# lichunshang/vision-enhanced-lidar-odometry

Hardware: AMD Instinct MI355X
Metric: scan-pairs/sec + achieved HBM GB/s, 120k-pt HDL-64E frame-to-frame ICP (higher is better)
Workload: dtype f32 association / f64 residuals+solve

## Files before the change

### vision-enhanced-lidar-odometry_amd/csrc/velo_kernels.h

```cpp
#pragma once
#include <hip/hip_runtime.h>
#include <stdint.h>

#include "velo_device_math.h"

#ifndef VELO_DEF_LOAD
#define VELO_DEF_LOAD 0
#endif
#ifndef VELO_DEF_ASSOC
#define VELO_DEF_ASSOC 0
#endif
#ifndef VELO_DEF_LMA
#define VELO_DEF_LMA 0
#endif
#ifndef VELO_DEF_LMB
#define VELO_DEF_LMB 0
#endif

namespace velo {

constexpr int kWave = 64;
constexpr int kNumAcc = 28;
constexpr int kEvalThreads = 256;
constexpr int kMaxEvalBlocks = 512;
// ... 2565 lines not shown
__device__ __forceinline__ int visual_block_eval3(const PoseEval& P, const VisualMatch& m, int slot, double& r0, double& r1, double& r2, double J[18]) {
    r0 = 0.0; r1 = 0.0; r2 = 0.0;
    int d;
    if (slot == 0) {
        if (!WITH_2D2D || (m.d1 && m.d2)) {
            const double a[3] = {m.p3_1[0], m.p3_1[1], m.p3_1[2]}, s[3] = {m.p3_2[0], m.p3_2[1], m.p3_2[2]};
            double rl[3];
            res_3d3d(P.fwd, P.t, a, s, rl, J);
            r0 = rl[0]; r1 = rl[1]; r2 = rl[2]; d = 3;
        } else {
            const double a[2] = {m.p2_1[0], m.p2_1[1]}, s[2] = {m.p2_2[0], m.p2_2[1]}, tc[3] = {m.t_cam[0], m.t_cam[1], m.t_cam[2]};
            double rl[1];
            res_2d2d(P.fwd, P.t, a, s, tc, rl, J);
            r0 = rl[0]; d = 1;
        }
    } else {
        const double tc[3] = {m.t_cam[0], m.t_cam[1], m.t_cam[2]};
        double rl[2];
        if (slot == 1) {
            const double a[3] = {m.p3_1[0], m.p3_1[1], m.p3_1[2]}, s[2] = {m.p2_2[0], m.p2_2[1]};
            res_3d2d(P.fwd, P.t, a, s, tc, rl, J);
        } else {
            const double a[3] = {m.p3_2[0], m.p3_2[1], m.p3_2[2]}, s[2] = {m.p2_1[0], m.p2_1[1]};
            res_2d3d(P.inv, P.t, a, s, tc, rl, J);
        }
        r0 = rl[0]; r1 = rl[1]; d = 2;
    }
    return d;
}
__device__ __forceinline__ int visual_block_eval(const PoseEval& P, const VisualMatch& m, int slot, double r[3], double J[18]) {
    double r0, r1, r2;
    const int d = visual_block_eval3(P, m, slot, r0, r1, r2, J);
    r[0] = r0; r[1] = r1; r[2] = r2;
    return d;
}

__device__ __forceinline__ void visual_gate_body(const double* __restrict__ xdev, const VisualParams& V, const VisualMatch* __restrict__ matches, int n, int iter,
                                                 unsigned char* __restrict__ flags, int* __restrict__ counts, const int i) {
    if (i >= n) return;
    double x[6];
#pragma unroll
    for (int k = 0; k < 6; k++) x[k] = xdev[k];
    PoseEval P;
    pose_eval_init(x, &P, true);
    const VisualMatch m = matches[i];
    unsigned char f0 = 0, f1 = 0, f2 = 0;
    bool stop = false;
    double r[3], J[18];
    const double it = (double)iter;
    if (m.d1 && m.d2) {
        visual_block_eval(P, m, 0, r, J);
        const double th2 = V.th_3d3d * V.outlier_reject / it * V.th_3d3d * V.outlier_reject / it;
        if (iter > 1 && r[0] * r[0] + r[1] * r[1] + r[2] * r[2] > th2) stop = true; else f0 = 1 + 0;
    }
    if (!stop && !m.d1 && !m.d2 && V.enable_2d2d) {
        visual_block_eval(P, m, 0, r, J);
        if (iter > 1 && fabs(r[0]) > V.th_2d2d * V.outlier_reject / it) stop = true; else f0 = 1 + 3;
    }
    if (V.enable_3d2d) {
        const double th2 = V.th_3d2d * V.outlier_reject / it * V.th_3d2d * V.outlier_reject / it;
        if (!stop && m.d1) {
            visual_block_eval(P, m, 1, r, J);
            if (iter > 1 && r[0] * r[0] + r[1] * r[1] > th2) stop = true; else f1 = 1 + 1;
        }
        if (!stop && m.d2) {
            visual_block_eval(P, m, 2, r, J);
            if (iter > 1 && r[0] * r[0] + r[1] * r[1] > th2) stop = true; else f2 = 1 + 2;
        }
    }
    flags[3 * i + 0] = f0; flags[3 * i + 1] = f1; flags[3 * i + 2] = f2;
    if (counts) {
        const int nb = (f0 ? 1 : 0) + (f1 ? 1 : 0) + (f2 ? 1 : 0);
        const int nr = (f0 ? (f0 - 1 == VELO_RESIDUAL_3D3D ? 3 : 1) : 0) + (f1 ? 2 : 0) + (f2 ? 2 : 0);
        if (nb) { atomicAdd(&counts[0], nb); atomicAdd(&counts[1], nr); }
    }
}
__global__ void visual_gate_kernel(const double* __restrict__ xdev, VisualParams V, const VisualMatch* __restrict__ matches, int n, int iter,
                                   unsigned char* __restrict__ flags, int* __restrict__ counts)
#if VELO_DEF_LMA
{
    visual_gate_body(xdev, V, matches, n, iter, flags, counts, (int)(blockIdx.x * blockDim.x + threadIdx.x));
}
#else
;
#endif
constexpr int kGateJobs = 8;
struct GateBatch {
    const double* x[kGateJobs]; const VisualMatch* m[kGateJobs]; unsigned char* flags[kGateJobs]; int* counts[kGateJobs]; int n[kGateJobs];
    VisualParams V; int iter;
};
__global__ void __launch_bounds__(128) visual_gate_batch_kernel(GateBatch G)
#if VELO_DEF_LMA
{
    const int j = blockIdx.y;
    visual_gate_body(G.x[j], G.V, G.m[j], G.n[j], G.iter, G.flags[j], G.counts[j], (int)(blockIdx.x * 128 + threadIdx.x));
}
#else
;
#endif

enum { PHASE_INIT = 0, PHASE_CAND = 1 };
struct LMParams {
    int max_num_iterations, max_invalid;
    double function_tolerance, gradient_tolerance, parameter_tolerance;
    double initial_radius, max_radius, min_radius, min_relative_decrease, min_diag, max_diag;
};
struct LMState {
    double x[6];
    double xc[6];
    double H[21];
    double g[6];
    double cost;
    double scale[6];
    double diag[6];
    double radius, decrease, x_norm, model_change, step_norm;
    double initial_cost;
    int reuse_diag, invalid, iter, evals, done, termination, phase, n_valid;
};
static_assert(sizeof(LMState) % 8 == 0 && sizeof(LMState) / 8 <= 64, "the state is copied by one wave, one 8-byte word per lane");

__device__ __forceinline__ int tri(int i, int j) { return i * 6 - (i * (i - 1)) / 2 + (j - i); }

struct LMEvalPoint {
    double M[4][9];
    double t[3];
    double x[6];
    int done;
    int pad;
};
static_assert(sizeof(LMEvalPoint) % 8 == 0 && sizeof(LMEvalPoint) / 8 <= 64, "the eval point is copied by one wave, one 8-byte word per lane");

__device__ __forceinline__ void eval_point_column(const double x[6], int done, int col, LMEvalPoint* P) {
    if (col < 3) {
        PoseRot R;
        pose_rot_init(x, &R);
        const double e[3] = {col == 0 ? 1.0 : 0.0, col == 1 ? 1.0 : 0.0, col == 2 ? 1.0 : 0.0};
        D3 m[3];
        rotate_point(R, e, m);
#pragma unroll
        for (int k = 0; k < 3; k++) {
            P->M[0][3 * k + col] = m[k].a;
#pragma unroll
            for (int j = 0; j < 3; j++) P->M[1 + j][3 * k + col] = m[k].v[j];
        }
    } else if (col == 3) {
#pragma unroll
        for (int k = 0; k < 3; k++) P->t[k] = x[3 + k];
#pragma unroll
        for (int k = 0; k < 6; k++) P->x[k] = x[k];
        P->done = done; P->pad = 0;
    }
}

__device__ __forceinline__ void res_3dpd_mat(const double (*M)[9], const double t[3], const double p[3], const double n[3], const double v0[3],
                                             double* r, double J[6]) {
    double m[3];
#pragma unroll
    for (int k = 0; k < 3; k++) m[k] = (M[0][3 * k] * p[0] + M[0][3 * k + 1] * p[1] + M[0][3 * k + 2] * p[2]) + (t[k] - v0[k]);
    *r = m[0] * n[0] + m[1] * n[1] + m[2] * n[2];
#pragma unroll
    for (int j = 0; j < 3; j++) {
        double d[3];
#pragma unroll
        for (int k = 0; k < 3; k++) d[k] = M[1 + j][3 * k] * p[0] + M[1 + j][3 * k + 1] * p[1] + M[1 + j][3 * k + 2] * p[2];
        J[j] = d[0] * n[0] + d[1] * n[1] + d[2] * n[2];
    }
    J[3] = n[0]; J[4] = n[1]; J[5] = n[2];
}

struct EvalArgs {
    const LMState* __restrict__ state;
    const LMEvalPoint* __restrict__ pt;
    const double* __restrict__ x_override;
    const float4* __restrict__ cp;
    const float4* __restrict__ cn;
    const float4* __restrict__ cv0;
    int q_begin, q_end;
    const VisualMatch* __restrict__ vm;
    const unsigned char* __restrict__ vflags;
    int n_matches;
    double loss_a_3dpd, w_3dpd;
    VisualParams V;
    double* __restrict__ partials;
    int vis_row0;
    double* __restrict__ rows_r;
    double* __restrict__ rows_J;
    const int* __restrict__ row_offset_vis;
    const int* __restrict__ row_offset_icp;
    unsigned long long* __restrict__ trace;
    int trace_eval;
};

constexpr int kStatTypes = 5;
constexpr int kStatBins = 65536;
struct StatWork {
    unsigned long long prefix[kStatTypes];
    long long k[kStatTypes];
    long long count[kStatTypes];
    double sum[kStatTypes];
    double cost;
};
__global__ void __launch_bounds__(256)
residual_norms_kernel(const double* __restrict__ xdev, EvalArgs A, double* __restrict__ vals, signed char* __restrict__ types,
                      double* __restrict__ part )
#if VELO_DEF_LMA
{
    __shared__ PoseEval s_P;
    __shared__ double s_red[256];
    if (threadIdx.x == 0) {
        double x[6];
        for (int k = 0; k < 6; k++) x[k] = xdev[k];
        pose_eval_init(x, &s_P, true);
    }
    __syncthreads();
    const int n_vis = 3 * A.n_matches, nq = A.q_end - A.q_begin;
    const int i = blockIdx.x * blockDim.x + threadIdx.x;
    double v = 0.0, sq = 0.0;
    int type = -1;
    if (i < n_vis) {
        const unsigned char f = A.vflags[i];
        if (f) {
            const VisualMatch m = A.vm[i / 3];
            double r0, r1, r2, J[18];
            const int d = visual_block_eval3(s_P, m, i % 3, r0, r1, r2, J);
            type = f - 1;
            if (d == 3) { sq = r0 * r0 + r1 * r1 + r2 * r2; v = sqrt(sq); }
            else if (d == 2) { sq = r0 * r0 + r1 * r1; v = sqrt(sq); }
            else { sq = r0 * r0; v = fabs(r0); }
        }
    } else if (i < n_vis + nq) {
        const int qi = A.q_begin + (i - n_vis);
        const float4 cp = A.cp[qi];
        if (__float_as_int(cp.w)) {
            const float4 cn = A.cn[qi], c0 = A.cv0[qi];
            const double p[3] = {cp.x, cp.y, cp.z}, n[3] = {cn.x, cn.y, cn.z}, v0[3] = {c0.x, c0.y, c0.z};
            double r, J[6];
            res_3dpd(s_P.fwd, s_P.t, p, n, v0, &r, J);
            type = VELO_FUNCTOR_3DPD; sq = r * r; v = fabs(r);
        }
    }
    if (i < n_vis + nq) { vals[i] = v; types[i] = (signed char)type; }
    for (int t = 0; t <= kStatTypes; t++) {
        s_red[threadIdx.x] = (t < kStatTypes) ? (type == t ? v : 0.0) : sq;
        __syncthreads();
        for (int off = 128; off > 0; off >>= 1) { if ((int)threadIdx.x < off) s_red[threadIdx.x] += s_red[threadIdx.x + off]; __syncthreads(); }
        if (threadIdx.x == 0) part[(size_t)blockIdx.x * (kStatTypes + 1) + t] = s_red[0];
        __syncthreads();
    }
}
#else
;
#endif
__global__ void __launch_bounds__(256)
stats_hist_kernel(const double* __restrict__ vals, const signed char* __restrict__ types, int n, int pass, const StatWork* __restrict__ W, int* __restrict__ hist)
#if VELO_DEF_LMA
{
    const int i = blockIdx.x * blockDim.x + threadIdx.x;
    if (i >= n) return;
    const int t = types[i];
    if (t < 0) return;
    const unsigned long long b = (unsigned long long)__double_as_longlong(vals[i]);
    if (pass > 0 && (b >> (64 - 16 * pass)) != W->prefix[t]) return;
    atomicAdd(&hist[(size_t)t * kStatBins + (int)((b >> (48 - 16 * pass)) & 0xffffull)], 1);
}
#else
;
#endif
__global__ void __launch_bounds__(256)
stats_pick_kernel(int pass, StatWork* __restrict__ W, int* __restrict__ hist)
#if VELO_DEF_LMA
{
    __shared__ long long s_tot[256];
    const int t = blockIdx.x, tid = threadIdx.x;
    int* h = hist + (size_t)t * kStatBins;
    constexpr int per = kStatBins / 256;
    long long mine = 0;
    for (int u = 0; u < per; u++) mine += h[tid * per + u];
    s_tot[tid] = mine;
    __syncthreads();
    if (tid == 0) {
        long long total = 0;
        for (int u = 0; u < 256; u++) total += s_tot[u];
        if (pass == 0) { W->count[t] = total; W->k[t] = total / 2; W->prefix[t] = 0ull; }
        long long k = W->k[t];
        if (total > 0) {
            int seg = 0;
            while (seg < 255 && k >= s_tot[seg]) { k -= s_tot[seg]; seg++; }
            int bin = seg * per;
            while (bin < seg * per + per - 1 && k >= h[bin]) { k -= h[bin]; bin++; }
            W->prefix[t] = (W->prefix[t] << 16) | (unsigned long long)bin;
            W->k[t] = k;
        }
    }
    __syncthreads();
    for (int u = 0; u < per; u++) h[tid * per + u] = 0;
}
#else
;
#endif
__global__ void stats_final_kernel(const double* __restrict__ part, int n_blocks, StatWork* __restrict__ W, velo_residual_stats* __restrict__ out)
#if VELO_DEF_LMA
{
    const int t = threadIdx.x;
    if (t > kStatTypes) return;
    double s = 0.0;
    for (int b = 0; b < n_blocks; b++) s += part[(size_t)b * (kStatTypes + 1) + t];
    if (t == kStatTypes) { out->cost = 0.5 * s; return; }
    const long long n = W->count[t];
    out->type[t].count = n;
    out->type[t].mean = n > 0 ? s / (double)n : 0.0;
    out->type[t].median = n > 0 ? __longlong_as_double((long long)W->prefix[t]) : 0.0;
}
#else
;
#endif

#ifdef VELO_DIAGNOSTICS
constexpr int kTraceMaxEvals = 64, kTraceStages = 16, kTraceWgs = 512;
__device__ __forceinline__ void lm_trace(unsigned long long* trace, int eval, int stage) {
    if (trace && threadIdx.x == 0 && eval < kTraceMaxEvals && (int)blockIdx.x < kTraceWgs)
        trace[((size_t)eval * kTraceStages + stage) * kTraceWgs + blockIdx.x] = __builtin_amdgcn_s_memrealtime();
}
#define VELO_LM_TRACE(trace, eval, stage) lm_trace(trace, eval, stage)
#else
#define VELO_LM_TRACE(trace, eval, stage) do { } while (0)
#endif

__device__ __forceinline__ void accumulate_row(double acc[kNumAcc], double r, const double Jr[6], double sr) {
    const double rk = r * sr;
    double J[6];
#pragma unroll
    for (int i = 0; i < 6; i++) J[i] = Jr[i] * sr;
    int k = 0;
#pragma unroll
    for (int i = 0; i < 6; i++) {
#pragma unroll
        for (int j = i; j < 6; j++) acc[k++] += J[i] * J[j];
    }
#pragma unroll
    for (int i = 0; i < 6; i++) acc[21 + i] += J[i] * rk;
}

constexpr int kScratchDoubles = 128 * kNumAcc;
#ifndef VELO_REDUCE_LDS
#define VELO_REDUCE_LDS 1
#endif
#if !VELO_REDUCE_LDS
__device__ __forceinline__ void block_reduce_store(double acc[kNumAcc], double* __restrict__ dst , double* __restrict__) {
    __shared__ double red[kEvalThreads / kWave][32];
    const int lane = threadIdx.x & 63, wid = threadIdx.x >> 6;
    double v[32];
#pragma unroll
    for (int k = 0; k < 32; k++) v[k] = (k < kNumAcc) ? acc[k] : 0.0;
#pragma unroll
    for (int n = 16, mask = 32; n >= 1; n >>= 1, mask >>= 1) {
        const bool hi = (lane & mask) != 0;
#pragma unroll
        for (int i = 0; i < n; i++) {
            const double mine = hi ? v[i + n] : v[i];
            const double send = hi ? v[i] : v[i + n];
            v[i] = mine + __shfl_xor(send, mask);
        }
    }
    v[0] += __shfl_xor(v[0], 1);
    const int idx = ((lane >> 5) & 1) * 16 + ((lane >> 4) & 1) * 8 + ((lane >> 3) & 1) * 4 + ((lane >> 2) & 1) * 2 + ((lane >> 1) & 1);
    if ((lane & 1) == 0) red[wid][idx] = v[0];
    __syncthreads();
    if (threadIdx.x < kNumAcc) {
        double t = 0.0;
#pragma unroll
        for (int w = 0; w < kEvalThreads / kWave; w++) t += red[w][threadIdx.x];
        dst[threadIdx.x] = t;
    }
}
#else
__device__ __forceinline__ void store_agent(double* p, double v) { __hip_atomic_store(p, v, __ATOMIC_RELAXED, __HIP_MEMORY_SCOPE_AGENT); }
__device__ __forceinline__ double load_agent(const double* p) { return __hip_atomic_load(p, __ATOMIC_RELAXED, __HIP_MEMORY_SCOPE_AGENT); }
template <bool COHERENT = false>
__device__ __forceinline__ void block_reduce_store(double acc[kNumAcc], double* __restrict__ dst , double* __restrict__ scratch, const int tid_in = -1) {
    constexpr int kCols = kEvalThreads / 4;
    static_assert(kNumAcc * kCols <= kScratchDoubles / 2, "scratch size");
    double (*red)[kCols] = reinterpret_cast<double (*)[kCols]>(scratch);
    __shared__ double red2[kNumAcc][8];
    const int t = tid_in < 0 ? (int)threadIdx.x : tid_in, lane = t & 63, wid = t >> 6;
#pragma unroll
    for (int k = 0; k < kNumAcc; k++) acc[k] += __shfl_xor(acc[k], 32);
#pragma unroll
    for (int k = 0; k < kNumAcc; k++) acc[k] += __shfl_xor(acc[k], 16);
    if (lane < 16) {
#pragma unroll
        for (int k = 0; k < kNumAcc; k++) red[k][wid * 16 + lane] = acc[k];
    }
    __syncthreads();
    if (t < kNumAcc * 8) {
        const int k = t >> 3, part = t & 7;
        double v = 0.0;
#pragma unroll
        for (int i = 0; i < kCols / 8; i++) v += red[k][part * (kCols / 8) + i];
        red2[k][part] = v;
    }
    __syncthreads();
    if (t < kNumAcc) {
        double v = 0.0;
#pragma unroll
        for (int i = 0; i < 8; i++) v += red2[t][i];
        if (COHERENT) store_agent(dst + t, v); else dst[t] = v;
    }
}
#endif

__device__ __forceinline__ bool eval_point_load(const EvalArgs& A, LMEvalPoint* s_pt) {
    if (A.x_override) {
        if (threadIdx.x < 4) {
            double x[6];
#pragma unroll
            for (int k = 0; k < 6; k++) x[k] = A.x_override[k];
            eval_point_column(x, 0, threadIdx.x, s_pt);
        }
    } else if (threadIdx.x < sizeof(LMEvalPoint) / 8) {
        reinterpret_cast<unsigned long long*>(s_pt)[threadIdx.x] = reinterpret_cast<const unsigned long long*>(A.pt)[threadIdx.x];
    }
    __syncthreads();
    return A.x_override || !s_pt->done;
}

constexpr int kPre = 4;
template <int PRE> struct RowPrefetchT { float4 p[PRE], n[PRE], v[PRE]; };
using RowPrefetch = RowPrefetchT<kPre>;
template <int PRE = kPre>
__device__ __forceinline__ RowPrefetchT<PRE> prefetch_rows(const EvalArgs& A, const int bx, const int nbx, const int tid_in = -1) {
    RowPrefetchT<PRE> f;
    const int tid = bx * blockDim.x + (tid_in < 0 ? (int)threadIdx.x : tid_in), nthreads = nbx * blockDim.x;
#pragma unroll
    for (int k = 0; k < PRE; k++) {
        const int i = min(A.q_begin + tid + k * nthreads, A.q_end - 1);
        f.p[k] = A.cp[i]; f.n[k] = A.cn[i]; f.v[k] = A.cv0[i];
    }
    return f;
}
template <bool M_FROM_LDS>
__device__ __forceinline__ void sweep_row(const EvalArgs& A, const LMEvalPoint& s_pt, const double (*Mreg)[9], const double t[3], const float4& p, const float4& n,
                                          const float4& v, const int i, double acc[kNumAcc]) {
    if (__float_as_int(p.w) == 0) return;
    const double (*M)[9] = M_FROM_LDS ? s_pt.M : Mreg;
    if (M_FROM_LDS) asm volatile("" : "+v"(M));
    const double pd[3] = {p.x, p.y, p.z}, nd[3] = {n.x, n.y, n.z}, vd[3] = {v.x, v.y, v.z};
    double r, J[6];
    res_3dpd_mat(M, t, pd, nd, vd, &r, J);
    double rho0, rho1;
    loss_cauchy(A.loss_a_3dpd, A.w_3dpd, r * r, &rho0, &rho1);
    acc[27] += 0.5 * rho0;
    const double sr = sqrt(rho1);
    accumulate_row(acc, r, J, sr);
    if (A.rows_r) {
        const int row = A.row_offset_icp[i];
        A.rows_r[row] = r * sr;
#pragma unroll
        for (int k = 0; k < 6; k++) A.rows_J[(size_t)row * 6 + k] = J[k] * sr;
    }
}
template <bool M_FROM_LDS, int PRE = kPre>
__device__ __forceinline__ void sweep_rows(const EvalArgs& A, const RowPrefetchT<PRE>& f, const LMEvalPoint& s_pt, const int bx, const int nbx, double acc[kNumAcc], const int tid_in = -1) {
    const int tid = bx * blockDim.x + (tid_in < 0 ? (int)threadIdx.x : tid_in), nthreads = nbx * blockDim.x;
    double Mreg[4][9];
    if (!M_FROM_LDS) {
#pragma unroll
        for (int a = 0; a < 4; a++) {
#pragma unroll
            for (int k = 0; k < 9; k++) Mreg[a][k] = s_pt.M[a][k];
        }
    }
    double t[3];
#pragma unroll
    for (int k = 0; k < 3; k++) t[k] = s_pt.t[k];
#pragma unroll
    for (int k = 0; k < kNumAcc; k++) acc[k] = 0.0;
#pragma unroll
    for (int k = 0; k < PRE; k++) {
        const int i = A.q_begin + tid + k * nthreads;
        if (i < A.q_end) sweep_row<M_FROM_LDS>(A, s_pt, Mreg, t, f.p[k], f.n[k], f.v[k], i, acc);
    }
    for (int i = A.q_begin + tid + PRE * nthreads; i < A.q_end; i += nthreads) sweep_row<M_FROM_LDS>(A, s_pt, Mreg, t, A.cp[i], A.cn[i], A.cv0[i], i, acc);
}

__device__ __forceinline__ void eval_icp_body(const EvalArgs& A, const int bx, const int nbx) {
    const RowPrefetch f = prefetch_rows(A, bx, nbx);
    VELO_LM_TRACE(A.trace, A.trace_eval, 0);
    __shared__ LMEvalPoint s_pt;
    if (!eval_point_load(A, &s_pt)) return;
    VELO_LM_TRACE(A.trace, A.trace_eval, 1);
    double acc[kNumAcc];
    sweep_rows<true>(A, f, s_pt, bx, nbx, acc);
    VELO_LM_TRACE(A.trace, A.trace_eval, 2);
#if VELO_REDUCE_LDS
    __shared__ double s_scratch[kScratchDoubles / 2];
#else
    double* s_scratch = nullptr;
#endif
    block_reduce_store(acc, A.partials + (size_t)bx * kNumAcc, s_scratch);
    VELO_LM_TRACE(A.trace, A.trace_eval, 3);
}

__global__ void __launch_bounds__(kEvalThreads)
eval_icp_kernel(EvalArgs A)
#if VELO_DEF_LMA
{ eval_icp_body(A, blockIdx.x, gridDim.x); }
#else
;
#endif

struct LMBatchItem {
    EvalArgs A;
    LMState* S;
    const double* xd;
    const int* n_valid;
    int nb_icp;
    int nb_vis;
    int n_rows;
    PoseRecord* pose_out;
    SolveLog* log;
};
__global__ void __launch_bounds__(kEvalThreads)
eval_icp_batch_kernel(const LMBatchItem* __restrict__ items)
#if VELO_DEF_LMA
{
    const LMBatchItem& it = items[blockIdx.y];
    if ((int)blockIdx.x >= it.nb_icp) return;
    eval_icp_body(it.A, blockIdx.x, it.nb_icp);
}
#else
;
#endif
__device__ __forceinline__ void visual_sweep_acc(const EvalArgs& A, const LMEvalPoint& pt, const int bx, const int nbx, double acc[kNumAcc]) {
    __shared__ PoseEval s_P;
    if (threadIdx.x == 0) {
        double x[6];
#pragma unroll
        for (int k = 0; k < 6; k++) x[k] = pt.x[k];
        pose_eval_init(x, &s_P, true);
    }
    __syncthreads();
    const PoseEval& P = s_P;
#pragma unroll
    for (int k = 0; k < kNumAcc; k++) acc[k] = 0.0;
    const int tid = bx * blockDim.x + threadIdx.x, nthreads = nbx * blockDim.x;
    for (int s = tid; s < 3 * A.n_matches; s += nthreads) {
        const unsigned char f = A.vflags[s];
        if (!f) continue;
        const int mi = s / 3, slot = s - 3 * mi;
        const VisualMatch m = A.vm[mi];
        double r0, r1, r2, J[18];
        const int d = visual_block_eval3(P, m, slot, r0, r1, r2, J);
        const double sq = r0 * r0 + (d > 1 ? r1 * r1 : 0.0) + (d > 2 ? r2 * r2 : 0.0);
        double rho0, rho1;
        const int type = f - 1;
        if (type == 0) loss_arctan(A.V.th_3d3d, 1.0, sq, &rho0, &rho1);
        else if (type == 3) loss_arctan(A.V.th_2d2d, A.V.w_2d2d, sq, &rho0, &rho1);
        else loss_arctan(A.V.th_3d2d, A.V.w_3d2d, sq, &rho0, &rho1);
        acc[27] += 0.5 * rho0;
        const double sr = sqrt(rho1);
        accumulate_row(acc, r0, J, sr);
        if (d > 1) accumulate_row(acc, r1, J + 6, sr);
        if (d > 2) accumulate_row(acc, r2, J + 12, sr);
        if (A.rows_r) {
            const int row = A.row_offset_vis[s];
            A.rows_r[row] = r0 * sr;
            if (d > 1) A.rows_r[row + 1] = r1 * sr;
            if (d > 2) A.rows_r[row + 2] = r2 * sr;
#pragma unroll
            for (int c = 0; c < 18; c++) if (c < 6 * d) A.rows_J[(size_t)row * 6 + c] = J[c] * sr;
        }
    }
}
__device__ __forceinline__ void visual_sweep_one(const EvalArgs& A, const LMEvalPoint& pt, const int bx, const int nbx, double acc[kNumAcc]) {
    __shared__ PoseEval s_P;
    if (threadIdx.x == 0) {
        double x[6];
#pragma unroll
        for (int k = 0; k < 6; k++) x[k] = pt.x[k];
        pose_eval_init(x, &s_P, true);
    }
    __syncthreads();
    const PoseEval& P = s_P;
    const int s = bx * blockDim.x + threadIdx.x;
    const unsigned char f = s < 3 * A.n_matches ? A.vflags[s] : (unsigned char)0;
    double r0 = 0.0, r1 = 0.0, r2 = 0.0, J[18], sr = 0.0, rho0 = 0.0;
    int d = 0;
#pragma unroll
    for (int c = 0; c < 18; c++) J[c] = 0.0;
    if (f) {
        const int mi = s / 3, slot = s - 3 * mi;
        const VisualMatch m = A.vm[mi];
        if (slot == 0 && !(m.d1 && m.d2)) {
            const double a[2] = {m.p2_1[0], m.p2_1[1]}, q[2] = {m.p2_2[0], m.p2_2[1]}, tc[3] = {m.t_cam[0], m.t_cam[1], m.t_cam[2]};
            double rr;
            res_2d2d_win<2, 0>(P.fwd, P.t, a, q, tc, &r0, J);
            res_2d2d_win<2, 2>(P.fwd, P.t, a, q, tc, &rr, J + 2);
            res_2d2d_win<2, 4>(P.fwd, P.t, a, q, tc, &rr, J + 4);
            d = 1;
        } else d = visual_block_eval3<false>(P, m, slot, r0, r1, r2, J);
        const double sq = r0 * r0 + (d > 1 ? r1 * r1 : 0.0) + (d > 2 ? r2 * r2 : 0.0);
        double rho1;
        const int type = f - 1;
        if (type == 0) loss_arctan(A.V.th_3d3d, 1.0, sq, &rho0, &rho1);
        else if (type == 3) loss_arctan(A.V.th_2d2d, A.V.w_2d2d, sq, &rho0, &rho1);
        else loss_arctan(A.V.th_3d2d, A.V.w_3d2d, sq, &rho0, &rho1);
        sr = sqrt(rho1);
    }
#pragma unroll
    for (int k = 0; k < kNumAcc; k++) acc[k] = 0.0;
    if (f) {
        acc[27] += 0.5 * rho0;
        accumulate_row(acc, r0, J, sr);
        if (d > 1) accumulate_row(acc, r1, J + 6, sr);
        if (d > 2) accumulate_row(acc, r2, J + 12, sr);
        if (A.rows_r) {
            const int row = A.row_offset_vis[s];
            A.rows_r[row] = r0 * sr;
            if (d > 1) A.rows_r[row + 1] = r1 * sr;
            if (d > 2) A.rows_r[row + 2] = r2 * sr;
#pragma unroll
            for (int c = 0; c < 18; c++) if (c < 6 * d) A.rows_J[(size_t)row * 6 + c] = J[c] * sr;
        }
    }
}
__device__ __forceinline__ void eval_visual_body(const EvalArgs& A, const int bx, const int nbx) {
    __shared__ LMEvalPoint s_pt;
    if (!eval_point_load(A, &s_pt)) return;
    double acc[kNumAcc];
    visual_sweep_acc(A, s_pt, bx, nbx, acc);
#if VELO_REDUCE_LDS
    __shared__ double s_scratch[kScratchDoubles / 2];
#else
    double* s_scratch = nullptr;
#endif
// ... 520 lines not shown
    for (int i = 0; i < 6; i++) { sc[i] = S->scale[i]; gs[i] = S->g[i] * sc[i]; }
    const double scr = S->scale[r];
#pragma unroll
    for (int c = 0; c < 6; c++) {
        const double h = S->H[r <= c ? tri(r, c) : tri(c, r)];
        hrow[c] = h * scr * sc[c];
    }
    const int ei = lane < 36 ? lane / 6 : 5, ej = lane < 36 ? lane % 6 : 5;
    const double hs_e = S->H[ei <= ej ? tri(ei, ej) : tri(ej, ei)] * S->scale[ei] * S->scale[ej];
    int iter = S->iter, invalid = S->invalid, reuse = S->reuse_diag;
    double radius = S->radius, decrease = S->decrease;
    double diag_r = S->diag[r];
    for (;;) {
        if (iter + 1 > Q.max_num_iterations) { if (lane == 0) { S->done = 1; S->termination = 1; } break; }
        if (radius < Q.min_radius) { if (lane == 0) { S->done = 1; S->termination = 0; } break; }
        iter++;
        if (!reuse) {
            double hdd = hrow[0];
#pragma unroll
            for (int c = 1; c < 6; c++) hdd = (r == c) ? hrow[c] : hdd;
            diag_r = fmin(fmax(hdd, Q.min_diag), Q.max_diag);
        }
        const double inv_radius = 1.0 / radius;
        const double dterm = diag_r * inv_radius;
        double L[6], inv[6];
        bool ok = true;
#pragma unroll
        for (int j = 0; j < 6; j++) {
            double sj = (r == j) ? hrow[j] + dterm : hrow[j];
#pragma unroll
            for (int k = 0; k < j; k++) sj -= L[k] * lane_get(L[k], j);
            const double d = lane_get(sj, j);
            if (!(d > 0.0) || !isfinite(d)) { ok = false; break; }
            const double ljj = sqrt(d);
            inv[j] = 1.0 / ljj;
            L[j] = (r == j) ? ljj : sj * inv[j];
        }
        double y[6];
        if (ok) {
            double acc = gs[0];
#pragma unroll
            for (int c = 1; c < 6; c++) acc = (r == c) ? gs[c] : acc;
            double z[6];
#pragma unroll
            for (int k = 0; k < 6; k++) {
                z[k] = lane_get(acc, k) * inv[k];
                acc -= L[k] * z[k];
            }
#pragma unroll
            for (int i = 5; i >= 0; i--) {
                double sv = z[i];
#pragma unroll
                for (int k = i + 1; k < 6; k++) sv -= lane_get(L[i], k) * y[k];
                y[i] = sv * inv[i];
            }
#pragma unroll
            for (int i = 0; i < 6; i++) ok = ok && isfinite(y[i]);
        }
        reuse = 1;
        double mc = 0.0, step[6];
        if (ok) {
            double gd = 0.0, dHd = 0.0;
#pragma unroll
            for (int i = 0; i < 6; i++) step[i] = -y[i];
            double si = step[0], sj = step[0];
#pragma unroll
            for (int c = 1; c < 6; c++) { si = (ei == c) ? step[c] : si; sj = (ej == c) ? step[c] : sj; }
            const double prod = si * hs_e * sj;
#pragma unroll
            for (int i = 0; i < 6; i++) gd += gs[i] * step[i];
#pragma unroll
            for (int l = 0; l < 36; l++) dHd += lane_get(prod, l);
            mc = -(gd + 0.5 * dHd);
            if (!(mc > 0.0)) ok = false;
        }
        if (!ok) {
            if (++invalid >= Q.max_invalid) { if (lane == 0) { S->done = 1; S->termination = 2; } break; }
            radius = radius / decrease; decrease *= 2.0; reuse = 1;
            continue;
        }
        invalid = 0;
        if (lane == 0) {
            double dn = 0.0;
#pragma unroll
            for (int i = 0; i < 6; i++) { const double d = step[i] * sc[i]; S->xc[i] = S->x[i] + d; dn += d * d; }
            S->step_norm = sqrt(dn);
            S->model_change = mc;
            S->phase = PHASE_CAND;
        }
        break;
    }
    if (lane < 6) S->diag[lane] = diag_r;
    if (lane == 0) { S->iter = iter; S->invalid = invalid; S->reuse_diag = reuse; S->radius = radius; S->decrease = decrease; }
}
__device__ __forceinline__ void lm_transition_wave(const LMParams& Q, LMState* sL, const double* E, int lane) {
    int need = 0;
    if (lane == 0) {
        LMState L = *sL;
        bool ns = false;
        lm_transition_local(Q, &L, E, &ns);
        *sL = L;
        need = ns ? 1 : 0;
    }
    __builtin_amdgcn_fence(__ATOMIC_RELEASE, "wavefront");
    __builtin_amdgcn_wave_barrier();
    __builtin_amdgcn_fence(__ATOMIC_ACQUIRE, "wavefront");
    need = __builtin_amdgcn_readfirstlane(need);
    if (need) lm_compute_step_wave(Q, sL, lane);
    __builtin_amdgcn_fence(__ATOMIC_RELEASE, "wavefront");
    __builtin_amdgcn_wave_barrier();
    __builtin_amdgcn_fence(__ATOMIC_ACQUIRE, "wavefront");
}

__global__ void __launch_bounds__(256)
lm_step_kernel(LMParams Q, LMState* S, LMEvalPoint* pt, const double* __restrict__ partials, int n_blocks, unsigned long long* trace, int trace_eval,
               PoseRecord* __restrict__ pose_out, SolveLog* __restrict__ log)
#if VELO_DEF_LMA
{
    lm_transition(Q, S, pt, partials, n_blocks, trace, trace_eval, nullptr, pose_out, log);
}
#else
;
#endif
__global__ void __launch_bounds__(256)
lm_step_peer_kernel(LMParams Q, LMState* S, LMEvalPoint* pt, const double* __restrict__ partials, int n_blocks, PeerComm C,
                    PoseRecord* __restrict__ pose_out, SolveLog* __restrict__ log)
#if VELO_DEF_LMA
{
    lm_transition(Q, S, pt, partials, n_blocks, nullptr, 0, &C, pose_out, log);
}
#else
;
#endif
__global__ void lm_begin_batch_kernel(const LMBatchItem* __restrict__ items)
#if VELO_DEF_LMA
{
    const LMBatchItem& it = items[blockIdx.x];
    lm_begin_body(it.S, const_cast<LMEvalPoint*>(it.A.pt), it.xd, it.n_valid);
    if (threadIdx.x == 0 && it.pose_out) it.pose_out->ready = 0;
}
#else
;
#endif
__global__ void __launch_bounds__(256)
lm_step_batch_kernel(LMParams Q, const LMBatchItem* __restrict__ items)
#if VELO_DEF_LMA
{
    const LMBatchItem& it = items[blockIdx.x];
    lm_transition(Q, it.S, const_cast<LMEvalPoint*>(it.A.pt), it.A.partials, it.n_rows, nullptr, 0, nullptr, it.pose_out, it.log);
}
#else
;
#endif
template <bool M_LDS, int PRE, int CHUNK, bool VIS = false>
__device__ __forceinline__ void eval_step_batch_body(const LMParams& Q, const LMBatchItem& it, int* __restrict__ tickets, const int first) {
    const int bx = blockIdx.x, nbx = it.nb_icp, nb_all = VIS ? it.nb_icp + it.nb_vis : it.nb_icp;
    if (bx >= nb_all) return;
#ifdef VELO_LM_SETPRIO
    __builtin_amdgcn_s_setprio(VELO_LM_SETPRIO);
#endif
    const EvalArgs& A = it.A;
    const RowPrefetchT<PRE> f = prefetch_rows<PRE>(A, (VIS && bx >= nbx) ? 0 : bx, nbx);
    __shared__ LMEvalPoint s_pt;
    __shared__ LMState sL;
    __shared__ double s_scratch[CHUNK * kNumAcc];
    __shared__ int s_last;
    static_assert(CHUNK * kNumAcc >= kScratchDoubles / 2, "the sweep's reduction needs 64 columns x 28");
    if (first) {
        if (threadIdx.x < 4) {
            double x[6];
#pragma unroll
            for (int k = 0; k < 6; k++) x[k] = it.xd ? it.xd[k] : it.S->x[k];
            eval_point_column(x, 0, threadIdx.x, &s_pt);
        }
        __syncthreads();
    } else
    if (!eval_point_load(A, &s_pt)) return;
    double acc[kNumAcc];
    if (VIS && bx >= nbx) {
        if (M_LDS) visual_sweep_one(A, s_pt, bx - nbx, it.nb_vis, acc);
        else visual_sweep_acc(A, s_pt, bx - nbx, it.nb_vis, acc);
        block_reduce_store<true>(acc, A.partials + (size_t)(A.vis_row0 + bx - nbx) * kNumAcc, s_scratch);
    } else {
        sweep_rows<M_LDS, PRE>(A, f, s_pt, bx, nbx, acc);
        block_reduce_store<true>(acc, A.partials + (size_t)bx * kNumAcc, s_scratch);
    }
    asm volatile("s_waitcnt vmcnt(0)" ::: "memory");
    __syncthreads();
    if (threadIdx.x == 0) s_last = __hip_atomic_fetch_add(tickets + blockIdx.y, 1, __ATOMIC_RELAXED, __HIP_MEMORY_SCOPE_AGENT) == nb_all - 1 ? 1 : 0;
    __syncthreads();
    if (!s_last) return;
    if (threadIdx.x == 0) __hip_atomic_store(tickets + blockIdx.y, 0, __ATOMIC_RELAXED, __HIP_MEMORY_SCOPE_AGENT);
    lm_advance<true, CHUNK, false, true>(Q, it.S, A.partials, it.n_rows, first ? 2 : 0, it.xd, it.n_valid, s_scratch, &sL, &s_pt, nullptr, 0, nullptr, it.pose_out, it.log);
    const int t = threadIdx.x;
    LMEvalPoint* pt = const_cast<LMEvalPoint*>(A.pt);
    if (t < (int)(sizeof(LMState) / 8)) reinterpret_cast<unsigned long long*>(it.S)[t] = reinterpret_cast<const unsigned long long*>(&sL)[t];
    else if (t >= 64 && t < 64 + (int)(sizeof(LMEvalPoint) / 8)) reinterpret_cast<unsigned long long*>(pt)[t - 64] = reinterpret_cast<const unsigned long long*>(&s_pt)[t - 64];
}
__global__ void __launch_bounds__(kEvalThreads)
eval_step_batch_kernel(LMParams Q, const LMBatchItem* __restrict__ items, int* __restrict__ tickets, int first)
#if VELO_DEF_LMB
{
    eval_step_batch_body<false, kPre, kStepChunk>(Q, items[blockIdx.y], tickets, first);
}
#else
;
#endif
#ifndef VELO_LEAN_PRE
#define VELO_LEAN_PRE 1
#endif
__global__ void __launch_bounds__(kEvalThreads) __attribute__((amdgpu_num_vgpr(152)))
eval_step_batch_lean_kernel(LMParams Q, const LMBatchItem* __restrict__ items, int* __restrict__ tickets, int first)
#if VELO_DEF_LMB
{
    eval_step_batch_body<true, VELO_LEAN_PRE, 64>(Q, items[blockIdx.y], tickets, first);
}
#else
;
#endif
__global__ void __launch_bounds__(kEvalThreads) __attribute__((amdgpu_num_vgpr(152)))
eval_step_batch_lean_vis_kernel(LMParams Q, const LMBatchItem* __restrict__ items, int* __restrict__ tickets, int first)
#if VELO_DEF_LMB
{
    eval_step_batch_body<true, VELO_LEAN_PRE, 64, true>(Q, items[blockIdx.y], tickets, first);
}
#else
;
#endif
__global__ void __launch_bounds__(kEvalThreads)
eval_step_batch_vis_kernel(LMParams Q, const LMBatchItem* __restrict__ items, int* __restrict__ tickets, int first)
#if VELO_DEF_LMB
{
    eval_step_batch_body<false, kPre, kStepChunk, true>(Q, items[blockIdx.y], tickets, first);
}
#else
;
#endif
struct LMBatchPackV { LMBatchItem item[4]; };
__global__ void __launch_bounds__(kEvalThreads)
eval_step_batch_v_kernel(LMParams Q, LMBatchPackV P, int* __restrict__ tickets, int first)
#if VELO_DEF_LMB
{
    eval_step_batch_body<false, kPre, kStepChunk>(Q, P.item[blockIdx.y], tickets, first);
}
#else
;
#endif
__global__ void __launch_bounds__(kEvalThreads) __attribute__((amdgpu_num_vgpr(152)))
eval_step_batch_lean_v_kernel(LMParams Q, LMBatchPackV P, int* __restrict__ tickets, int first)
#if VELO_DEF_LMB
{
    eval_step_batch_body<true, VELO_LEAN_PRE, 64>(Q, P.item[blockIdx.y], tickets, first);
}
#else
;
#endif
__global__ void __launch_bounds__(kEvalThreads) __attribute__((amdgpu_num_vgpr(152)))
eval_step_batch_lean_vis_v_kernel(LMParams Q, LMBatchPackV P, int* __restrict__ tickets, int first)
#if VELO_DEF_LMB
{
    eval_step_batch_body<true, VELO_LEAN_PRE, 64, true>(Q, P.item[blockIdx.y], tickets, first);
}
#else
;
#endif
template <bool M_LDS, int PRE, int CHUNK>
__device__ __forceinline__ void lm_iter_lean_body(const EvalArgs& A, const LMParams& Q, const LMState* __restrict__ Sin, LMState* __restrict__ Sout,
                                                  const double* __restrict__ pin, int n_in, double* __restrict__ pout, int first,
                                                  const double* __restrict__ x_in, const int* __restrict__ n_valid, const int bx, const int nbx,
                                                  PoseRecord* pose_out, SolveLog* log) {
    __shared__ LMState sL;
    __shared__ LMEvalPoint s_pt;
    __shared__ double s_scratch[CHUNK * kNumAcc];
    const RowPrefetchT<PRE> f = prefetch_rows<PRE>(A, bx, nbx);
    lm_advance<false, CHUNK>(Q, Sin, pin, n_in, first, x_in, n_valid, s_scratch, &sL, &s_pt, nullptr, 0, nullptr, pose_out, log, bx == 0);
    const int t = threadIdx.x;
    if (bx == 0 && t < (int)(sizeof(LMState) / 8)) reinterpret_cast<unsigned long long*>(Sout)[t] = reinterpret_cast<const unsigned long long*>(&sL)[t];
    if (sL.done) return;
    double acc[kNumAcc];
    sweep_rows<M_LDS, PRE>(A, f, s_pt, bx, nbx, acc);
    block_reduce_store(acc, pout + (size_t)bx * kNumAcc, s_scratch);
}
__global__ void __launch_bounds__(kEvalThreads) __attribute__((amdgpu_num_vgpr(152)))
lm_iter_batch_lean_kernel(LMParams Q, LMBatchPackV P, int parity, int first, size_t half)
#if VELO_DEF_LMB
{
    const LMBatchItem& it = P.item[blockIdx.y];
    if ((int)blockIdx.x >= it.nb_icp) return;
    lm_iter_lean_body<true, VELO_LEAN_PRE, 64>(it.A, Q, it.S + parity, it.S + (parity ^ 1), it.A.partials + (size_t)parity * half, it.nb_icp,
                                               it.A.partials + (size_t)(parity ^ 1) * half, first, it.xd, it.n_valid, blockIdx.x, it.nb_icp, it.pose_out, it.log);
}
#else
;
#endif
__device__ __forceinline__ int ctl_load(const int* p) { return __hip_atomic_load(p, __ATOMIC_RELAXED, __HIP_MEMORY_SCOPE_AGENT); }
__device__ __forceinline__ void ctl_store(int* p, int v) { __hip_atomic_store(p, v, __ATOMIC_RELAXED, __HIP_MEMORY_SCOPE_AGENT); }
#ifndef VELO_TEST_ATTR
#define VELO_TEST_ATTR __attribute__((amdgpu_num_vgpr(152)))
#endif
struct AgCtl { int epoch, abort, pad[30]; int flag[2][kMaxEvalBlocks]; };

struct SolveCtl { int ticket, pad0[31]; int arrived, pad1[31]; int gen, pad2[31]; int exited, pad3[31]; };
constexpr int kSolveDone = 1 << 30;
template <int PRE>
__device__ __forceinline__ int persist_sweep(const EvalArgs& A, SolveCtl* __restrict__ ctl, const int k, const int bx, const int nb,
                                             LMEvalPoint* s_pt, double* s_scratch, int* s_flag) {
    const int t = threadIdx.x;
    const LMEvalPoint* pt = A.pt;
    const RowPrefetchT<PRE> f = prefetch_rows<PRE>(A, bx, nb);
    if (t == 0) {
        int fl = 0;
        for (;;) {
            const int g = ctl_load(&ctl->gen);
            if (g & kSolveDone) { fl = 1; break; }
            if (g > k) break;
            __builtin_amdgcn_s_sleep(8);
        }
        *s_flag = fl;
    }
    __syncthreads();
    const int over = *s_flag;
    __syncthreads();
    if (over) return -1;
    if (t < (int)(sizeof(LMEvalPoint) / 8))
        reinterpret_cast<unsigned long long*>(s_pt)[t] = __hip_atomic_load(reinterpret_cast<const unsigned long long*>(pt) + t, __ATOMIC_RELAXED, __HIP_MEMORY_SCOPE_AGENT);
    __syncthreads();
    double acc[kNumAcc];
#ifndef VELO_T2
    sweep_rows<true, PRE>(A, f, *s_pt, bx, nb, acc);
#else
    for (int q = 0; q < kNumAcc; q++) acc[q] = f.p[0].x;
#endif
    block_reduce_store<true>(acc, A.partials + (size_t)bx * kNumAcc, s_scratch);
    asm volatile("s_waitcnt vmcnt(0)" ::: "memory");
    __syncthreads();
    if (t == 0) *s_flag = __hip_atomic_fetch_add(&ctl->arrived, 1, __ATOMIC_RELAXED, __HIP_MEMORY_SCOPE_AGENT) == nb - 1 ? 1 : 0;
    __syncthreads();
    const int last = *s_flag;
    __syncthreads();
    return last;
}
__device__ __attribute__((noinline)) void persist_advance(const LMParams* Q, const LMBatchItem* it, int first, double* s_scratch, LMState* sL, LMEvalPoint* s_pt) {
    lm_advance<true, 64, true>(*Q, it->S, it->A.partials, it->n_rows, first, it->xd, it->n_valid, s_scratch, sL, s_pt, nullptr, 0, nullptr, it->pose_out, it->log);
}
template <int PRE>
__device__ __forceinline__ void lm_solve_persist_body(const LMParams& Q, const LMBatchItem* __restrict__ item, SolveCtl* __restrict__ ctl, const int kmax, const int n_wgs) {
    __shared__ LMEvalPoint s_pt;
    __shared__ LMState sL;
    __shared__ double s_scratch[64 * kNumAcc];
    __shared__ int s_ticket, s_flag;
    const int t = threadIdx.x;
    bool running = true;
    while (running) {
        const LMBatchItem* itp = item;
        asm volatile("" : "+s"(itp));
        const LMBatchItem& it = *itp;
        const EvalArgs& A = it.A;
        const int nb = it.nb_icp;
        LMEvalPoint* pt = const_cast<LMEvalPoint*>(A.pt);
        if (t == 0) s_ticket = __hip_atomic_fetch_add(&ctl->ticket, 1, __ATOMIC_RELAXED, __HIP_MEMORY_SCOPE_AGENT);
        __syncthreads();
        const int tk = s_ticket;
        __syncthreads();
        const int k = (tk - 1) / nb, bx = (tk - 1) - k * nb;
        int advance = 0;
        if (tk == 0) advance = 1;
        else if (k >= kmax) running = false;
        else {
            const int r = persist_sweep<PRE>(A, ctl, k, bx, nb, &s_pt, s_scratch, &s_flag);
            if (r < 0) running = false;
            else if (r > 0) advance = 2;
        }
        if (advance) {
            if (advance == 2 && t == 0) ctl_store(&ctl->arrived, 0);
#ifndef VELO_T1
            persist_advance(&Q, itp, advance == 1 ? 1 : 0, s_scratch, &sL, &s_pt);
#endif
            if (t < (int)(sizeof(LMState) / 8)) __hip_atomic_store(reinterpret_cast<unsigned long long*>(it.S) + t, reinterpret_cast<const unsigned long long*>(&sL)[t], __ATOMIC_RELAXED, __HIP_MEMORY_SCOPE_AGENT);
            else if (t >= 64 && t < 64 + (int)(sizeof(LMEvalPoint) / 8)) __hip_atomic_store(reinterpret_cast<unsigned long long*>(pt) + (t - 64), reinterpret_cast<const unsigned long long*>(&s_pt)[t - 64], __ATOMIC_RELAXED, __HIP_MEMORY_SCOPE_AGENT);
            asm volatile("s_waitcnt vmcnt(0)" ::: "memory");
            __syncthreads();
            if (t == 0) ctl_store(&ctl->gen, (advance == 1 ? 1 : k + 2) | (sL.done ? kSolveDone : 0));
            __syncthreads();
        }
    }
    __syncthreads();
    if (t == 0 && __hip_atomic_fetch_add(&ctl->exited, 1, __ATOMIC_RELAXED, __HIP_MEMORY_SCOPE_AGENT) == n_wgs - 1) {
        ctl_store(&ctl->ticket, 0); ctl_store(&ctl->arrived, 0); ctl_store(&ctl->gen, 0); ctl_store(&ctl->exited, 0);
    }
}
__global__ void __launch_bounds__(kEvalThreads, 3)
lm_solve_persist_batch_kernel(LMParams Q, const LMBatchItem* __restrict__ items, SolveCtl* __restrict__ ctl, int kmax)
#if VELO_DEF_LMB
{
    lm_solve_persist_body<VELO_LEAN_PRE>(Q, items + blockIdx.y, ctl + blockIdx.y, kmax, (int)gridDim.x);
}
#else
;
#endif

__global__ void lm_gather_states_kernel(const LMBatchItem* __restrict__ items, LMState* __restrict__ out, int which)
#if VELO_DEF_LMB
{
    const unsigned* src = reinterpret_cast<const unsigned*>(items[blockIdx.x].S + which);
    unsigned* dst = reinterpret_cast<unsigned*>(out + blockIdx.x);
    for (int k = threadIdx.x; k < (int)(sizeof(LMState) / 4); k += blockDim.x) dst[k] = src[k];
}
#else
;
#endif

constexpr int kFinishJobs = 8;
struct ChainFinish {
    const LMState* S[kFinishJobs];
    const unsigned char* vflags[kFinishJobs]; const int* vis_counts[kFinishJobs];
    unsigned char* h_vflags[kFinishJobs]; int* h_vis_counts[kFinishJobs];
    int n_vflags[kFinishJobs];
    const SolveLog* logs; const int* fail;
    LMState* h_states; SolveLog* h_logs; int* h_fail;
    int n, n_logs, n_counts;
};
__global__ void __launch_bounds__(256) chain_finish_kernel(ChainFinish F)
#if VELO_DEF_LMB
{
    const int i = blockIdx.x, t = threadIdx.x;
    {
        const unsigned* src = reinterpret_cast<const unsigned*>(F.S[i]);
        unsigned* dst = reinterpret_cast<unsigned*>(F.h_states + i);
        for (int k = t; k < (int)(sizeof(LMState) / 4); k += 256) dst[k] = src[k];
    }
    {
        const unsigned* src = reinterpret_cast<const unsigned*>(F.logs + (size_t)i * F.n_logs);
        unsigned* dst = reinterpret_cast<unsigned*>(F.h_logs + (size_t)i * F.n_logs);
        for (int k = t; k < (int)(sizeof(SolveLog) / 4) * F.n_logs; k += 256) dst[k] = src[k];
    }
    if (t == 0) F.h_fail[i] = F.fail[i];
    if (F.n_vflags[i] > 0) {
        for (int k = t; k < F.n_vflags[i]; k += 256) F.h_vflags[i][k] = F.vflags[i][k];
        for (int k = t; k < F.n_counts; k += 256) F.h_vis_counts[i][k] = F.vis_counts[i][k];
    }
}
#else
;
#endif

constexpr int kSmallRows = 4;
template <bool VIS = true>
__device__ __forceinline__ void
lm_solve_small_body(const EvalArgs& A, const LMParams& Q, LMState* Sg, const double* __restrict__ x_in, const int* __restrict__ n_valid,
                    int nb_icp, int nb_vis, int max_sweeps, PoseRecord* __restrict__ pose_out, SolveLog* __restrict__ log) {
    __shared__ double rows[kSmallRows][kNumAcc];
    __shared__ double part[8][kNumAcc];
    __shared__ double E[kNumAcc];
    __shared__ double s_x[6];
    __shared__ LMState sL;
    __shared__ int s_done;
    const int t = threadIdx.x;
    if (t == 0) {
        LMState L = *Sg;
        if (x_in) for (int i = 0; i < 6; i++) L.x[i] = x_in[i];
        L.n_valid = n_valid ? *n_valid : 0;
        L.phase = PHASE_INIT; L.done = 0; L.termination = 1; L.iter = 0; L.evals = 0; L.invalid = 0; L.reuse_diag = 0;
        sL = L;
        for (int i = 0; i < 6; i++) s_x[i] = L.x[i];
        s_done = 0;
        if (pose_out) pose_out->ready = 0;
    }
    __syncthreads();
    EvalArgs B = A;
    B.x_override = s_x;
    B.partials = &rows[0][0];
    B.vis_row0 = nb_icp;
    const int n_rows = nb_icp + nb_vis;
    for (int sweep = 0; sweep < max_sweeps; sweep++) {
        if (s_done) break;
        for (int bx = 0; bx < nb_icp; bx++) eval_icp_body(B, bx, nb_icp);
        if (VIS) for (int bx = 0; bx < nb_vis; bx++) eval_visual_body(B, bx, nb_vis);
        __syncthreads();
        if (t < 8 * kNumAcc) {
            const int k = t % kNumAcc, p = t / kNumAcc;
            double v = 0.0;
            for (int b = p; b < n_rows; b += 8) v += rows[b][k];
// ... 178 lines not shown
```

### vision-enhanced-lidar-odometry_amd/csrc/velo_lm_ag_kernels.h

```cpp
#pragma once
#include "velo_kernels.h"

namespace velo {

#ifndef VELO_AG_KATTR
#define VELO_AG_KATTR
#endif
#ifndef VELO_AG_PRE
#define VELO_AG_PRE VELO_LEAN_PRE
#endif
#ifndef VELO_AG_WAVES
#define VELO_AG_WAVES 3
#endif
#ifndef VELO_AG_NOINLINE
#define VELO_AG_NOINLINE __forceinline__
#endif
constexpr unsigned long long kAgTimeoutTicks = 2000000ull;
__device__ __forceinline__ bool ag_wait(AgCtl* __restrict__ ctl, const int parity, const int nb, const int tag, const int abort_tag, const int tid) {
    bool ok = true;
    const unsigned long long t0 = __builtin_amdgcn_s_memrealtime();
    for (int i = tid; i < nb; i += kEvalThreads) {
        while ((int)(ctl_load(&ctl->flag[parity][i]) - tag) < 0) {
            __builtin_amdgcn_s_sleep(4);
            if (__builtin_amdgcn_s_memrealtime() - t0 > kAgTimeoutTicks || ctl_load(&ctl->abort) == abort_tag) { ok = false; break; }
        }
        if (!ok) break;
    }
    const int all = __syncthreads_and(ok ? 1 : 0);
    if (!all && tid == 0) ctl_store(&ctl->abort, abort_tag);
    return all != 0;
}
template <int CHUNK>
__device__ VELO_AG_NOINLINE void ag_advance(const LMParams* Q, const LMState* S, const double* xd, const int* n_valid, PoseRecord* pose_out, SolveLog* log,
                                                    const double* partials, int nb, int first, double* s_scratch, LMState* sL, LMEvalPoint* s_pt, bool writer, int tid) {
    lm_advance<true, CHUNK, false, true>(*Q, S, partials, nb, first ? 2 : 0, xd, n_valid, s_scratch, sL, s_pt, nullptr, 0, nullptr, pose_out, log, writer, first != 0, tid);
}
template <bool M_LDS, int PRE, int CHUNK>
__device__ __forceinline__ void lm_solve_ag_body(const LMParams& Q, const LMBatchItem& it, AgCtl* __restrict__ ctl, const int kmax, const size_t half) {
    __shared__ LMEvalPoint s_pt;
    __shared__ LMState sL;
    __shared__ double s_scratch[CHUNK * kNumAcc];
    const int t = threadIdx.x, bx = blockIdx.x;
    const int nb = it.nb_icp;
    if (bx >= nb) return;
    const int epoch = ctl->epoch;
    {
        if (t < 4) {
            double x[6];
#pragma unroll
            for (int k = 0; k < 6; k++) x[k] = it.xd ? it.xd[k] : it.S->x[k];
            eval_point_column(x, 0, t, &s_pt);
        }
        __syncthreads();
    }
    bool finished = false;
    RowPrefetchT<PRE> f = prefetch_rows<PRE>(it.A, bx, nb);
#pragma clang loop unroll(disable)
    for (int k = 0; k < kmax; k++) {
        int tt = t;
        asm volatile("" : "+v"(tt));
        const EvalArgs& A = it.A;
        double acc[kNumAcc];
        sweep_rows<M_LDS, PRE>(A, f, s_pt, bx, nb, acc, tt);
        block_reduce_store<true>(acc, A.partials + (size_t)(k & 1) * half + (size_t)bx * kNumAcc, s_scratch, tt);
        asm volatile("s_waitcnt vmcnt(0)" ::: "memory");
        __syncthreads();
        if (tt == 0) ctl_store(&ctl->flag[k & 1][bx], epoch + k + 1);
#ifdef VELO_AG_PREFETCH
        f = prefetch_rows<PRE>(A, bx, nb, tt);
#endif
        if (!ag_wait(ctl, k & 1, nb, epoch + k + 1, epoch + 1, tt)) break;
        ag_advance<CHUNK>(&Q, it.S, it.xd, it.n_valid, it.pose_out, it.log, A.partials + (size_t)(k & 1) * half, nb, k == 0 ? 1 : 0, s_scratch, &sL, &s_pt, bx == 0, tt);
        if (sL.done) { finished = true; break; }
#ifndef VELO_AG_PREFETCH
        f = prefetch_rows<PRE>(A, bx, nb, tt);
#endif
    }
    if (bx == 0) {
        if (finished && t < (int)(sizeof(LMState) / 8)) reinterpret_cast<unsigned long long*>(it.S)[t] = reinterpret_cast<const unsigned long long*>(&sL)[t];
        if (t == 0) ctl->epoch = epoch + kmax + 4;
    }
}
__global__ void __launch_bounds__(kEvalThreads, VELO_AG_WAVES) VELO_AG_KATTR
lm_solve_ag_batch_kernel(LMParams Q, LMBatchPackV P, AgCtl* __restrict__ ctl, int kmax, size_t half) {
    lm_solve_ag_body<true, VELO_AG_PRE, 64>(Q, P.item[blockIdx.y], ctl + blockIdx.y, kmax, half);
}


}
```

Before: 4219.

## Batch row loads into chunks and use LDS address space for pose matrix

The tail loop of the ICP residual sweep now issues the loads for three rows at once and then processes them, so several global loads are in flight per thread instead of one dependent load per row. When the prefetch depth is below the default, it also requests the first chunk before sweeping the prefetched rows. The pose matrix pointer is cast to the LDS address space so the compiler can emit ds_read instead of flat loads. A new slim kernel variant keeps the old per-row loop under a VGPR cap. The chunking raises register pressure, which may reduce occupancy.

```diff
diff --git a/vision-enhanced-lidar-odometry_amd/csrc/velo_kernels.h b/vision-enhanced-lidar-odometry_amd/csrc/velo_kernels.h
--- a/vision-enhanced-lidar-odometry_amd/csrc/velo_kernels.h
+++ b/vision-enhanced-lidar-odometry_amd/csrc/velo_kernels.h
@@ -2741,7 +2741,8 @@
     }
 }
 
-__device__ __forceinline__ void res_3dpd_mat(const double (*M)[9], const double t[3], const double p[3], const double n[3], const double v0[3],
+template <class MatPtr>
+__device__ __forceinline__ void res_3dpd_mat(const MatPtr M, const double t[3], const double p[3], const double n[3], const double v0[3],
                                              double* r, double J[6]) {
     double m[3];
 #pragma unroll
@@ -3031,11 +3032,14 @@
 __device__ __forceinline__ void sweep_row(const EvalArgs& A, const LMEvalPoint& s_pt, const double (*Mreg)[9], const double t[3], const float4& p, const float4& n,
                                           const float4& v, const int i, double acc[kNumAcc]) {
     if (__float_as_int(p.w) == 0) return;
-    const double (*M)[9] = M_FROM_LDS ? s_pt.M : Mreg;
-    if (M_FROM_LDS) asm volatile("" : "+v"(M));
     const double pd[3] = {p.x, p.y, p.z}, nd[3] = {n.x, n.y, n.z}, vd[3] = {v.x, v.y, v.z};
     double r, J[6];
-    res_3dpd_mat(M, t, pd, nd, vd, &r, J);
+    if (M_FROM_LDS) {
+        typedef const __attribute__((address_space(3))) double (*LdsMat)[9];
+        LdsMat M = (LdsMat)s_pt.M;
+        asm volatile("" : "+v"(M));
+        res_3dpd_mat(M, t, pd, nd, vd, &r, J);
+    } else res_3dpd_mat(Mreg, t, pd, nd, vd, &r, J);
     double rho0, rho1;
     loss_cauchy(A.loss_a_3dpd, A.w_3dpd, r * r, &rho0, &rho1);
     acc[27] += 0.5 * rho0;
@@ -3048,7 +3052,22 @@
         for (int k = 0; k < 6; k++) A.rows_J[(size_t)row * 6 + k] = J[k] * sr;
     }
 }
-template <bool M_FROM_LDS, int PRE = kPre>
+constexpr int kRowChunk = 3;
+struct RowChunk { float4 p[kRowChunk], n[kRowChunk], v[kRowChunk]; };
+__device__ __forceinline__ void row_chunk_request(const EvalArgs& A, const int i0, const int nthreads, RowChunk& g) {
+#pragma unroll
+    for (int k = 0; k < kRowChunk; k++) {
+        const int i = min(i0 + k * nthreads, A.q_end - 1);
+        g.p[k] = A.cp[i]; g.n[k] = A.cn[i]; g.v[k] = A.cv0[i];
+    }
+}
+__device__ __forceinline__ void row_chunk_arrive(RowChunk& g) {
+#pragma unroll
+    for (int k = 0; k < kRowChunk; k++)
+        asm volatile("" : "+v"(g.p[k].x), "+v"(g.p[k].y), "+v"(g.p[k].z), "+v"(g.p[k].w), "+v"(g.n[k].x), "+v"(g.n[k].y), "+v"(g.n[k].z),
+                          "+v"(g.v[k].x), "+v"(g.v[k].y), "+v"(g.v[k].z));
+}
+template <bool M_FROM_LDS, int PRE = kPre, bool AHEAD = (PRE < kPre), bool TOGETHER = true>
 __device__ __forceinline__ void sweep_rows(const EvalArgs& A, const RowPrefetchT<PRE>& f, const LMEvalPoint& s_pt, const int bx, const int nbx, double acc[kNumAcc], const int tid_in = -1) {
     const int tid = bx * blockDim.x + (tid_in < 0 ? (int)threadIdx.x : tid_in), nthreads = nbx * blockDim.x;
     double Mreg[4][9];
@@ -3064,12 +3083,27 @@
     for (int k = 0; k < 3; k++) t[k] = s_pt.t[k];
 #pragma unroll
     for (int k = 0; k < kNumAcc; k++) acc[k] = 0.0;
+    int i0 = A.q_begin + tid + PRE * nthreads;
+    RowChunk g;
+    if (AHEAD && TOGETHER) row_chunk_request(A, i0, nthreads, g);
 #pragma unroll
     for (int k = 0; k < PRE; k++) {
         const int i = A.q_begin + tid + k * nthreads;
         if (i < A.q_end) sweep_row<M_FROM_LDS>(A, s_pt, Mreg, t, f.p[k], f.n[k], f.v[k], i, acc);
     }
-    for (int i = A.q_begin + tid + PRE * nthreads; i < A.q_end; i += nthreads) sweep_row<M_FROM_LDS>(A, s_pt, Mreg, t, A.cp[i], A.cn[i], A.cv0[i], i, acc);
+    if (!TOGETHER) {
+        for (int i = i0; i < A.q_end; i += nthreads) sweep_row<M_FROM_LDS>(A, s_pt, Mreg, t, A.cp[i], A.cn[i], A.cv0[i], i, acc);
+        return;
+    }
+    for (bool requested = AHEAD; requested || i0 < A.q_end; requested = false, i0 += kRowChunk * nthreads) {
+        if (!requested) row_chunk_request(A, i0, nthreads, g);
+        row_chunk_arrive(g);
+#pragma unroll
+        for (int k = 0; k < kRowChunk; k++) {
+            const int i = i0 + k * nthreads;
+            if (i < A.q_end) sweep_row<M_FROM_LDS>(A, s_pt, Mreg, t, g.p[k], g.n[k], g.v[k], i, acc);
+        }
+    }
 }
 
 __device__ __forceinline__ void eval_icp_body(const EvalArgs& A, const int bx, const int nbx) {
@@ -3896,7 +3930,7 @@
 #else
 ;
 #endif
-template <bool M_LDS, int PRE, int CHUNK, bool VIS = false>
+template <bool M_LDS, int PRE, int CHUNK, bool VIS = false, bool ROWS_TOGETHER = true>
 __device__ __forceinline__ void eval_step_batch_body(const LMParams& Q, const LMBatchItem& it, int* __restrict__ tickets, const int first) {
     const int bx = blockIdx.x, nbx = it.nb_icp, nb_all = VIS ? it.nb_icp + it.nb_vis : it.nb_icp;
     if (bx >= nb_all) return;
@@ -3926,7 +3960,7 @@
         else visual_sweep_acc(A, s_pt, bx - nbx, it.nb_vis, acc);
         block_reduce_store<true>(acc, A.partials + (size_t)(A.vis_row0 + bx - nbx) * kNumAcc, s_scratch);
     } else {
-        sweep_rows<M_LDS, PRE>(A, f, s_pt, bx, nbx, acc);
+        sweep_rows<M_LDS, PRE, (PRE < kPre), ROWS_TOGETHER>(A, f, s_pt, bx, nbx, acc);
         block_reduce_store<true>(acc, A.partials + (size_t)bx * kNumAcc, s_scratch);
     }
     asm volatile("s_waitcnt vmcnt(0)" ::: "memory");
@@ -3995,6 +4029,15 @@
 #if VELO_DEF_LMB
 {
     eval_step_batch_body<true, VELO_LEAN_PRE, 64>(Q, P.item[blockIdx.y], tickets, first);
+}
+#else
+;
+#endif
+__global__ void __launch_bounds__(kEvalThreads) __attribute__((amdgpu_num_vgpr(152)))
+eval_step_batch_lean_v_slim_kernel(LMParams Q, LMBatchPackV P, int* __restrict__ tickets, int first)
+#if VELO_DEF_LMB
+{
+    eval_step_batch_body<true, VELO_LEAN_PRE, 64, false, false>(Q, P.item[blockIdx.y], tickets, first);
 }
 #else
 ;
@@ -4071,7 +4114,7 @@
     __syncthreads();
     double acc[kNumAcc];
 #ifndef VELO_T2
-    sweep_rows<true, PRE>(A, f, *s_pt, bx, nb, acc);
+    sweep_rows<true, PRE, false>(A, f, *s_pt, bx, nb, acc);
 #else
     for (int q = 0; q < kNumAcc; q++) acc[q] = f.p[0].x;
 #endif
diff --git a/vision-enhanced-lidar-odometry_amd/csrc/velo_lm_ag_kernels.h b/vision-enhanced-lidar-odometry_amd/csrc/velo_lm_ag_kernels.h
--- a/vision-enhanced-lidar-odometry_amd/csrc/velo_lm_ag_kernels.h
+++ b/vision-enhanced-lidar-odometry_amd/csrc/velo_lm_ag_kernels.h
@@ -61,7 +61,7 @@
         asm volatile("" : "+v"(tt));
         const EvalArgs& A = it.A;
         double acc[kNumAcc];
-        sweep_rows<M_LDS, PRE>(A, f, s_pt, bx, nb, acc, tt);
+        sweep_rows<M_LDS, PRE, false>(A, f, s_pt, bx, nb, acc, tt);
         block_reduce_store<true>(acc, A.partials + (size_t)(k & 1) * half + (size_t)bx * kNumAcc, s_scratch, tt);
         asm volatile("s_waitcnt vmcnt(0)" ::: "memory");
         __syncthreads();
```

Result: faster. 4339, median of 6 (+2.8%).
